# klkuhlm/unconfined

Hardware: AMD Instinct MI355X
Metric: (t,r) drawdown points/sec, Neuman-1974 1024x256 sweep; max |rel err| vs CPU ref (higher is better)
Workload: dtype f64

## Files before the change

unconfined_amd/csrc/ucf_device.h:

```cpp

#include "ucf_math.h"
#include "ucf_plan.h"
#include <type_traits>

namespace UCF_NS {

using namespace ucfm;

#define UCF_STR_(x) #x
#define UCF_STR(x) UCF_STR_(x)
#define UCF_PI 3.14159265358979323846
#define UCF_EPS 2.220446049250313e-16

UCF_DEV double shfl_down1(double v) { return __shfl_down(v, 1, 64); }
UCF_DEV double shift_down1(double x)
{
    const int lo = __double2loint(x), hi = __double2hiint(x);
    const int l2 = __builtin_amdgcn_update_dpp(lo, lo, 0x130, 0xf, 0xf, false);
    const int h2 = __builtin_amdgcn_update_dpp(hi, hi, 0x130, 0xf, 0xf, false);
    return __hiloint2double(h2, l2);
}
UCF_DEV cplx shfl_down1(cplx v) { return cmake(shift_down1(v.re), shift_down1(v.im)); }
UCF_DEV cplx bcast0(cplx v) { return cmake(__shfl(v.re, 0, 64), __shfl(v.im, 0, 64)); }
UCF_DEV double wave_max(double v)
// ... 608 lines not shown
#if UCF_FAST && UCF_DH_PACK
UCF_DEV cplx lane_gather(cplx v, int src) { return cmake(__shfl(v.re, src, 64), __shfl(v.im, src, 64)); }
template <int W>
UCF_DEV cplx qd_quotient_groups(cplx qn, cplx enn, cplx enew, bool valid, int lane)
{
    const double m = fmax(fabs(enew.re), fabs(enew.im));
    const unsigned long long bal = __builtin_amdgcn_ballot_w64(valid && !(m < 1.0e150 && m > 1.0e-150));
    const double r = fast_rcp(__builtin_fma(enew.re, enew.re, enew.im * enew.im));
    const cplx num = cmul(qn, enn);
    cplx res = cmake((num.re * enew.re + num.im * enew.im) * r, (num.im * enew.re - num.re * enew.im) * r);
    if (__builtin_expect(bal != 0, 0)) {
        const bool mine = ((bal >> (lane & ~(W - 1))) & ((1ull << W) - 1)) != 0;
        const cplx scaled = cdiv(cmul(qn, enn), enew);
        if (mine) res = scaled;
    }
    return res;
}
template <int W>
UCF_DEV void qd_step(cplx& q, cplx& en, int r, int M, int lane, bool occ, lds_c* dcol, int pitch)
{
    const int l = lane & (W - 1);
    const cplx qn = shfl_down1(q);
    const cplx enew = cadd(csub(qn, q), en);
    if (l == 0 && occ) {
        dcol[(size_t)(2 * r - 1) * pitch] = make_double2(-q.re, -q.im);
        dcol[(size_t)(2 * r) * pitch] = make_double2(-enew.re, -enew.im);
    }
    if (r < M) {
        const cplx enn = shfl_down1(enew);
        const bool valid = occ && l <= 2 * (M - r - 1) + 1;
        if constexpr (W == UCF_WAVE) q = qd_quotient(qn, enn, enew, valid);
        else q = qd_quotient_groups<W>(qn, enn, enew, valid, lane);
        en = enn;
    }
}
UCF_DEV void dehoog_qd_tile(const ucf_dev_params& P, int lane, int ncur, const double* __restrict__ tD4, lds_c* lds, lds_c* tileB,
                            int pitch, int* zflag, ucf_stats* st)
{
    const int M = P.M, np = P.np;
    const int r32 = (M - 15 > 1) ? M - 15 : 1, r16 = (M - 7 > 1) ? M - 7 : 1;
    const cplx c0 = cmake(0.0, 0.0);
    for (int tq = 0; tq < ncur; tq += 2) {
        cplx Qq = c0, Qe = c0;
        int present = 0;
        for (int hf = 0; hf < 2 && tq + hf < ncur; hf++) {
            const int tt = tq + hf;
            const double tee = 2.0 * tD4[tt];
            const double sigma = P.alpha - P.logtol / (2.0 * tee);
            cplx tl = c0;
            if (lane < np) { const lds_c v = lds[lane * pitch + tt]; tl = cmake(v.x, v.y); }
            const cplx p = cmake(sigma, UCF_PI * lane / tee);
            cplx Pq = c0, Pe = c0;
            for (int which = 0; which < 2; which++) {
                lds_c* col = (which ? tileB : lds) + tt;
                cplx q;
                const bool some = qd_start(which ? cmul(tl, p) : tl, M, lane, st, col, &q);
                const bool live = __builtin_amdgcn_ballot_w64(some) != 0;
                if (lane == 0) zflag[2 * tt + which] = !live;
                if (!live) continue;
                cplx en = c0;
                for (int r = 1; r < r32; r++) qd_step<UCF_WAVE>(q, en, r, M, lane, true, col, pitch);
                present |= 1 << (2 * hf + which);
                const cplx gq = lane_gather(q, lane & 31), ge = lane_gather(en, lane & 31);
                if ((lane >> 5) == which) { Pq = gq; Pe = ge; }
            }
            if (((present >> (2 * hf)) & 3) == 0) continue;
            {
                const int g = lane >> 5;
                const bool occ = (present >> (2 * hf + g)) & 1;
                lds_c* col = (g ? tileB : lds) + tt;
                for (int r = r32; r < r16; r++) qd_step<32>(Pq, Pe, r, M, lane, occ, col, pitch);
                const int src = ((lane >> 4) & 1) * 32 + (lane & 15);
                const cplx gq = lane_gather(Pq, src), ge = lane_gather(Pe, src);
                if ((lane >> 5) == hf) { Qq = gq; Qe = ge; }
            }
        }
        if (present == 0) continue;
        const int g = lane >> 4;
        const bool occ = (present >> g) & 1;
        lds_c* col = ((g & 1) ? tileB : lds) + tq + (g >> 1);
        for (int r = r16; r <= M; r++) qd_step<16>(Qq, Qe, r, M, lane, occ, col, pitch);
    }
}
#endif

UCF_DEV double dehoog_cf_lane(const lds_c* dcol, int pitch, int M, double alpha, double logtol, double t, double tee)
{
    const double gamma = alpha - logtol / (2.0 * tee);
    const lds_c v0 = dcol[0];
    const cplx d0 = cmake(v0.x, v0.y);
    cplx Am2 = cmake(0.0, 0.0), Am1 = d0, Bm2 = cmake(1.0, 0.0), Bm1 = cmake(1.0, 0.0);
    const cplx z = cexp_(cdivr(cscale(cscale(cmake(0.0, 1.0), UCF_PI), t), tee));
    for (int n = 1; n <= 2 * M - 1; n++) {
        const lds_c v = dcol[(size_t)n * pitch];
        const cplx d = cmake(v.x, v.y);
        const cplx An = cadd(Am1, cmul(cmul(d, Am2), z));
        const cplx Bn = cadd(Bm1, cmul(cmul(d, Bm2), z));
        Am2 = Am1; Am1 = An; Bm2 = Bm1; Bm1 = Bn;
    }
    const lds_c vq = dcol[(size_t)(2 * M - 1) * pitch], ve = dcol[(size_t)(2 * M) * pitch];
    const cplx dlast_q = cmake(vq.x, vq.y), dlast_e = cmake(ve.x, ve.y);
    const cplx brem = cdivr(radd(1.0, cmul(csub(dlast_q, dlast_e), z)), 2.0);
    const cplx inner = csqrt_(radd(1.0, cdiv(cmul(dlast_e, z), cmul(brem, brem))));
    const cplx rem = cneg(cmul(brem, rsub(1.0, inner)));
    const cplx A2M = cadd(Am1, cmul(rem, Am2));
    const cplx B2M = cadd(Bm1, cmul(rem, Bm2));
    return exp(gamma * t) / tee * cdiv(A2M, B2M).re;
}

template <int G>
UCF_DEV void shift_down_sets(const cplx (&in)[G], cplx (&out)[G], int lane)
{
#pragma unroll
    for (int g = 0; g < G; g++) {
        const cplx a = shfl_down1(in[g]);
        const cplx nx = (g + 1 < G) ? bcast0(in[g + 1 < G ? g + 1 : g]) : a;
        out[g] = (lane == 63 && g + 1 < G) ? nx : a;
    }
}

template <int G>
UCF_DEV double dehoog_sets(const cplx (&f)[G], int M, double alpha, double logtol, double t, double tee, int lane,
                           ucf_stats* st)
{
    const int n2 = 2 * M;
    double mag = 0.0;
    cplx ff[G], q[G], e[G];
    bool nans[G];
#pragma unroll
    for (int g = 0; g < G; g++) {
        const int i = lane + 64 * g;
        const bool act = i <= n2;
        double m1 = act ? cabs_(f[g]) : 0.0;
        if (d_isnan(m1)) m1 = 0.0;
        mag = fmax(mag, m1);
        const bool nanp = act && (d_isnan(f[g].re) || d_isnan(f[g].im));
        nans[g] = nanp;
        ff[g] = (nanp || !act) ? cmake(act ? 0.0 : 1.0, 0.0) : f[g];
    }
    const double mx = wave_max(mag);
    if (!(mx > UCF_DBL_MIN)) {
        if (st) stat_add(&st->zero_vectors, lane == 0);
        return 0.0;
    }
    if (st) {
#pragma unroll
        for (int g = 0; g < G; g++) stat_add(&st->nan_scrubbed, nans[g]);
    }
    const double gamma = alpha - logtol / (2.0 * tee);
    const cplx ff0 = bcast0(ff[0]);
    const cplx d0 = cdivr(ff0, 2.0);
    cplx fn[G];
    shift_down_sets<G>(ff, fn, lane);
#pragma unroll
    for (int g = 0; g < G; g++) {
        const int i = lane + 64 * g;
        q[g] = (i == 0) ? cdiv(fn[g], d0) : cdiv(fn[g], ff[g]);
        if (i > n2 - 1) q[g] = cmake(1.0, 0.0);
        e[g] = cmake(0.0, 0.0);
    }
    cplx Am2 = cmake(0.0, 0.0), Am1 = d0, Bm2 = cmake(1.0, 0.0), Bm1 = cmake(1.0, 0.0);
    const cplx z = cexp_(cdivr(cscale(cscale(cmake(0.0, 1.0), UCF_PI), t), tee));
    cplx dlast_q = cmake(0.0, 0.0), dlast_e = cmake(0.0, 0.0);
    for (int r = 1; r <= M; r++) {
        cplx qn[G], en[G], enew[G];
        shift_down_sets<G>(q, qn, lane);
        shift_down_sets<G>(e, en, lane);
#pragma unroll
        for (int g = 0; g < G; g++) {
            const int i = lane + 64 * g;
            enew[g] = cadd(csub(qn[g], q[g]), en[g]);
            if (i > 2 * (M - r)) enew[g] = cmake(1.0, 0.0);
        }
        const cplx dq = cneg(bcast0(q[0]));
        const cplx de = cneg(bcast0(enew[0]));
        {
            cplx An = cadd(Am1, cmul(cmul(dq, Am2), z));
            cplx Bn = cadd(Bm1, cmul(cmul(dq, Bm2), z));
            Am2 = Am1; Am1 = An; Bm2 = Bm1; Bm1 = Bn;
        }
        if (r < M) {
            cplx An = cadd(Am1, cmul(cmul(de, Am2), z));
            cplx Bn = cadd(Bm1, cmul(cmul(de, Bm2), z));
            Am2 = Am1; Am1 = An; Bm2 = Bm1; Bm1 = Bn;
            cplx enn[G];
            shift_down_sets<G>(enew, enn, lane);
#pragma unroll
            for (int g = 0; g < G; g++) {
                const int i = lane + 64 * g;
                q[g] = cdiv(cmul(qn[g], enn[g]), enew[g]);
                if (i > 2 * (M - r - 1) + 1) q[g] = cmake(1.0, 0.0);
// ... 824 lines not shown
                } else {
                    cplx acc = cadd(lds_ld(accCur, z, lane), cscale(val, P.tab_premul ? 1.0 : P.gl_w[m]));
                    if (m == ngl - 1) {
                        const double lob = P.j0z[sv + jj - 1] / rD;
                        const double hib = P.j0z[sv + jj] / rD;
                        acc = rscale((hib - lob) / 2.0, acc);
                        areas[(size_t)(jj * nz + z) * UCF_WAVE + lane] = make_double2(acc.re, acc.im);
                        acc = cmake(0.0, 0.0);
                    }
                    lds_st(accCur, z, lane, acc);
                }
            }
            if (!ts && ++m == ngl) { m = 0; jj++; }
        }
        for (int s = 0; s < (R + 1) * nz; s++) sti[(size_t)s * UCF_WAVE + lane] = lds[s * UCF_WAVE + lane];
        if (lane == 0) ndone[pt] = nabs;
    }
}

template <int LAYOUT, int PART, bool WREG, int MODE = 0>
__global__ void __launch_bounds__(UCF_WAVE, (LAYOUT == 0 || (WREG && MODE != 1)) ? 3 : 4)
finish_kernel(const ucf_dev_params P, int npts, int per_point, int nr, int nsv, int svmin,
              const double* __restrict__ tDv, const double* __restrict__ rDv, const int* __restrict__ svv,
              double* __restrict__ hout, double* __restrict__ dhout, ucf_stats* st, int nt, int ir0,
              double2* __restrict__ totlap, const double2* __restrict__ state, const int* __restrict__ ndone, int* __restrict__ defer)
{
    extern __shared__ lds_c lds[];
    const int lane = threadIdx.x;
    const int nz = P.nz, R = P.R, nacc = P.nacc;
    const int nabs = P.N + nacc * P.ngl;
    lds_c* accTS = lds;
    lds_c* scr = lds + (size_t)R * nz * UCF_WAVE;
    const int nloop = (MODE == 2) ? defer[0] : npts;
    for (int wi = blockIdx.x; wi < nloop; wi += gridDim.x) {
        const int pt = (MODE == 2) ? defer[1 + wi] / nz : wi;
        const int zsel = (MODE == 2) ? defer[1 + wi] % nz : 0;
        if (MODE != 2 && ndone[pt] < nabs) continue;
        const work_item W = decode_item<LAYOUT>(P, pt, lane, per_point, nr, nt, ir0, npts);
        const double tD = tDv[W.it], rD = rDv[W.ir];
        const int sv = (LAYOUT == 1) ? svmin : svv[W.it];
        const double tee = 2.0 * tD;
        const double sigma = P.alpha - P.logtol / (2.0 * tee);
        const cplx p = cmake(sigma, UCF_PI * W.mlap / tee);
        const double arg = P.j0z[sv - 1] / rD;
        const double2* __restrict__ sti = state + (size_t)pt * state_slots(P) * UCF_WAVE;
        for (int s = 0; s < R * nz; s++) lds[s * UCF_WAVE + lane] = sti[(size_t)s * UCF_WAVE + lane];
        finish_item<LAYOUT, PART, WREG, MODE>(P, accTS, scr, nullptr, sti + (size_t)(R + 1) * nz * UCF_WAVE, arg, W, pt, tD, tee, p, st, nt, ir0,
                                              totlap, hout, dhout, zsel, (MODE == 2) ? zsel + 1 : nz, (MODE == 1) ? defer : nullptr);
    }
}

#ifndef UCF_DH_TILE
#define UCF_DH_TILE 4
#endif
#if UCF_TU_HAS(1) || UCF_TU_HAS(3)
#ifndef UCF_DH_WAVES
#define UCF_DH_WAVES 4
#endif
template <int TU, bool BIG>
__global__ void __launch_bounds__(UCF_WAVE, BIG ? 4 : UCF_DH_WAVES)
dehoog_tiles_kernel(const ucf_dev_params P, int nt, int nr, int ir0, int nrc, const double* __restrict__ tDv,
                    const double2* __restrict__ totlap, double* __restrict__ hout, double* __restrict__ dhout,
                    ucf_stats* st)
{
    extern __shared__ lds_c lds[];
    const int lane = threadIdx.x;
    const int nz = P.nz, np = P.np;
    const int ntile = (nt + UCF_DH_TILE - 1) / UCF_DH_TILE;
    const long long nwork = (long long)nrc * ntile;
    const int pitch = UCF_DH_TILE + 1;
    lds_c* tileB = lds + (size_t)np * pitch;
    int* zflag = (int*)(tileB + (size_t)np * pitch);
    for (long long w = blockIdx.x; w < nwork; w += gridDim.x) {
        const int irl = (int)(w / ntile), it0 = (int)(w % ntile) * UCF_DH_TILE;
        const int ncur = (nt - it0 < UCF_DH_TILE) ? nt - it0 : UCF_DH_TILE;
        for (int z = 0; z < nz; z++) {
            const double2* src = totlap + ((size_t)irl * nz + z) * np * nt;
            for (int e = lane; e < np * UCF_DH_TILE; e += UCF_WAVE) {
                const int m = e / UCF_DH_TILE, tt = e % UCF_DH_TILE;
                if (tt < ncur) lds[m * pitch + tt] = src[(size_t)m * nt + it0 + tt];
            }
            __syncthreads();
            if constexpr (!BIG) {
#if UCF_FAST && UCF_DH_PACK
                dehoog_qd_tile(P, lane, ncur, tDv + it0, lds, tileB, pitch, zflag, st);
#else
                for (int tt = 0; tt < ncur; tt++) {
                    const double tD = tDv[it0 + tt];
                    const double tee = 2.0 * tD;
                    const double sigma = P.alpha - P.logtol / (2.0 * tee);
                    cplx tl = cmake(0.0, 0.0);
                    if (lane < np) { const lds_c v = lds[lane * pitch + tt]; tl = cmake(v.x, v.y); }
                    const cplx p = cmake(sigma, UCF_PI * lane / tee);
                    bool z0, z1;
                    dehoog_qd_wave(tl, P.M, lane, st, &z0, lds + tt, pitch);
                    dehoog_qd_wave(cmul(tl, p), P.M, lane, st, &z1, tileB + tt, pitch);
                    if (lane == 0) { zflag[2 * tt] = z0; zflag[2 * tt + 1] = z1; }
                }
#endif
                __syncthreads();
                if (lane < 2 * ncur) {
                    const int tt = lane >> 1, which = lane & 1;
                    const int it = it0 + tt;
                    const double tD = tDv[it];
                    double val = 0.0;
                    if (!zflag[lane]) val = dehoog_cf_lane((which ? tileB : lds) + tt, pitch, P.M, P.alpha, P.logtol, tD, 2.0 * tD);
                    const size_t o = ((size_t)it * nr + ir0 + irl) * P.nz_out + P.z_off + z;
                    if (which) dhout[o] = val * tD;
                    else hout[o] = val;
                }
            } else {
                for (int tt = 0; tt < ncur; tt++) {
                    const int it = it0 + tt;
                    const double tD = tDv[it];
                    const double tee = 2.0 * tD;
                    const double sigma = P.alpha - P.logtol / (2.0 * tee);
                    double hval, dval;
                    auto ld = [&](int i) { const lds_c v = lds[i * pitch + tt]; return cmake(v.x, v.y); };
                    if (np <= 2 * UCF_WAVE) dehoog_big<2>(ld, np, P.M, P.alpha, P.logtol, sigma, tD, tee, lane, st, &hval, &dval);
                    else dehoog_big<4>(ld, np, P.M, P.alpha, P.logtol, sigma, tD, tee, lane, st, &hval, &dval);
                    if (lane == 0) {
                        const size_t o = ((size_t)it * nr + ir0 + irl) * P.nz_out + P.z_off + z;
                        hout[o] = hval;
                        dhout[o] = dval;
                    }
                }
            }
            __syncthreads();
        }
    }
}

#endif

#if UCF_TU_HAS(2)
__global__ void __launch_bounds__(UCF_WAVE)
dehoog_points_kernel(const ucf_dev_params P, long long npc, int flat, int per_point, int nr, int ir0, int nrc,
                     const double* __restrict__ tDv, const double2* __restrict__ totlap, double* __restrict__ hout,
                     double* __restrict__ dhout, ucf_stats* st)
{
    const int lane = threadIdx.x;
    const int nz = P.nz;
    for (long long lp = blockIdx.x; lp < npc; lp += gridDim.x) {
        int it;
        size_t obase;
        if (flat) {
            it = per_point ? (int)lp : (int)(lp / nr);
            obase = (size_t)lp;
        } else {
            it = (int)(lp / nrc);
            obase = (size_t)it * nr + ir0 + (int)(lp % nrc);
        }
        const double tD = tDv[it];
        const double tee = 2.0 * tD;
        const double sigma = P.alpha - P.logtol / (2.0 * tee);
        for (int z = 0; z < nz; z++) {
            const double2* src = totlap + ((size_t)lp * nz + z) * P.np;
            double hval, dval;
            if (P.np <= UCF_WAVE) {
                const cplx p = cmake(sigma, UCF_PI * lane / tee);
                cplx tl = cmake(0.0, 0.0);
                if (lane < P.np) { const double2 v = src[lane]; tl = cmake(v.x, v.y); }
                hval = dehoog_wave(tl, P.M, P.alpha, P.logtol, tD, tee, lane, st);
                dval = dehoog_wave(cmul(tl, p), P.M, P.alpha, P.logtol, tD, tee, lane, st) * tD;
            } else {
                auto ld = [&](int i) { const double2 v = src[i]; return cmake(v.x, v.y); };
                if (P.np <= 2 * UCF_WAVE) dehoog_big<2>(ld, P.np, P.M, P.alpha, P.logtol, sigma, tD, tee, lane, st, &hval, &dval);
                else dehoog_big<4>(ld, P.np, P.M, P.alpha, P.logtol, sigma, tD, tee, lane, st, &hval, &dval);
            }
            if (lane == 0) {
                hout[obase * P.nz_out + P.z_off + z] = hval;
                dhout[obase * P.nz_out + P.z_off + z] = dval;
            }
        }
    }
}

#endif

template <int FAMILY>
__global__ void __launch_bounds__(UCF_WAVE)
samples_kernel(const ucf_dev_params P, int n_a, const double* __restrict__ av, double rD,
               const double* __restrict__ pv, double* __restrict__ fp)
{
    extern __shared__ lds_c lds[];
    const int lane = threadIdx.x;
    const int ia = blockIdx.x;
    if (ia >= n_a) return;
    const bool live = lane < P.np;
    const cplx p = live ? cmake(pv[2 * lane], pv[2 * lane + 1]) : cmake(1.0, 0.0);
    const double a = av[ia];
    bool need_lay1 = false;
    for (int z = 0; z < P.nz; z++) need_lay1 |= (P.zLay[z] == 1);
// ... 195 lines not shown
```

unconfined_amd/csrc/ucf_fastpath.h:

```cpp
#pragma once

namespace UCF_NS {

#define UCF_UNIFORM_BLOCK() asm volatile("" ::: "memory")
#define UCF_UNIFORM_BLOCK_F(FAMILY) do { if constexpr ((FAMILY) != 4) UCF_UNIFORM_BLOCK(); } while (0)

struct fprim {
    double ch, sh, ei, sn, cs;
};

template <bool POS, bool SMALLY = false>
UCF_DEV fprim prim_from_e(double x, double ax, double e, double ei, double y, const sc_ctx& sc)
{
    const int salt = sc.salt;
    fprim f;
    f.ei = ei;
    const double he = 0.5 * e;
    f.ch = __builtin_fma(0.5, ei, he);
    double s;
    if (ax < 0.35) {
        const double x2 = ax * ax;
        double pl = addk(mulk(x2, UCF_KHERE(1.0 / 6227020800.0, salt)), UCF_KHERE(1.0 / 39916800.0, salt));
        pl = fmak(pl, x2, UCF_KHERE(1.0 / 362880.0, salt));
        pl = fmak(pl, x2, UCF_KHERE(1.0 / 5040.0, salt));
// ... 74 lines not shown
    const double xz = xc * zD;
    const double e = exp_tab_(xc, sc), ez = exp_tab_(xz, sc);
    const double r = fast_rcp(e * ez);
    *f = prim_from_e<true, true>(xc, xc, e, r * ez, y, sc);
    *fz = prim_from_e<true, true>(xz, xz, ez, r * e, y * zD, sc);
}

UCF_DEV cplx cfma(cplx a, cplx b, cplx c)
{
    return cmake(__builtin_fma(a.re, b.re, __builtin_fma(-a.im, b.im, c.re)), __builtin_fma(a.re, b.im, __builtin_fma(a.im, b.re, c.im)));
}
UCF_DEV cplx cfnma(cplx a, cplx b, cplx c)
{
    return cmake(__builtin_fma(-a.re, b.re, __builtin_fma(a.im, b.im, c.re)), __builtin_fma(-a.re, b.im, __builtin_fma(-a.im, b.re, c.im)));
}
UCF_DEV cplx cinv_plain(cplx z)
{
    const double r = fast_rcp(z.re * z.re + z.im * z.im);
    return cmake(z.re * r, -(z.im * r));
}
UCF_DEV cplx cinv_scaled(cplx z)
{
    const double m = fmax(fabs(z.re), fabs(z.im));
    const int il = __builtin_amdgcn_frexp_exp(m) - 1;
    const double c = ldexp(z.re, -il), d = ldexp(z.im, -il);
    const double r = fast_rcp(c * c + d * d);
    return cmake(ldexp(c * r, -il), ldexp(-(d * r), -il));
}

UCF_DEV cplx cinv_auto(cplx z)
{
    const double m = fmax(fabs(z.re), fabs(z.im));
    if (__builtin_amdgcn_ballot_w64(!(m < 1.0e150 && m > 1.0e-150)) == 0) return cinv_plain(z);
    return cinv_scaled(z);
}

struct lane_consts {
    cplx p, lt, xifac;
    cplx fdB1;
    cplx mnpv;
};

UCF_DEV lane_consts make_lane_consts(const ucf_dev_params& P, cplx p, cplx lt)
{
    lane_consts L;
    L.p = p;
    L.lt = lt;
    cplx xf = rscale(P.alphaD, cinv_plain(p));
    if (P.model == 3) {
        cplx sum = cmake(0.0, 0.0);
        for (int j = 0; j < P.MoenchM; j++) sum = cadd(sum, cinv_plain(radd(1.0, cscale(p, P.MoenchInvGamma[j]))));
        xf = cmul(cscale(xf, (double)P.MoenchM), cinv_plain(sum));
    }
    L.xifac = xf;
    L.fdB1 = cscale(cscale(cscale(p, P.fd_beta0), P.fd_expmb2), P.inv_kappa);
    L.mnpv = radd(1.0, cscale(p, P.mn_vartheta * P.mn_c3));
    return L;
}

struct fast_common {
    sc_ctx sc;
    cplx th, eta, ff1, ff2, inv_she, she, che, top, g3, inv_den, ex1;
    cplx chz0;
    fprim p1;
    int have_p1;
    cplx mn_uod;
#ifdef UCF_SINGLE_RCP
    cplx q, den;
#endif
    cplx fd_s1;
    cplx top3, fd_s13;
    bool small_eta, fd_use, fd_use3;
    int any_small, any_large;
};

template <int FAMILY>
UCF_DEV double fast_scale(const ucf_dev_params& P)
{
    if (FAMILY == 0 || FAMILY == 3) return 2.0;
    if (FAMILY == 5) return P.inv_bD;
    return (FAMILY == 2 && P.model == 4) ? 2.0 : 2.0 * P.inv_bD;
}

template <int FAMILY, bool PAIR = false>
UCF_DEV bool fast_eta(const ucf_dev_params& P, const lane_consts& L, double a, fast_common& S)
{
    const double a2 = a * a;
    const cplx q = caddr(L.p, a2);
#ifdef UCF_SINGLE_RCP
    S.q = q;
#endif
    double mq = 0.0;
    if (PAIR && FAMILY != 0) {
        double r;
        rsq_pair(q.re * q.re + q.im * q.im, &mq, &r);
        S.th = cmake(q.re * r, -(q.im * r));
    } else {
        const double r = fast_rcp(q.re * q.re + q.im * q.im);
        S.th = cmake(q.re * r, -(q.im * r));
    }
    if (FAMILY == 0) return q.re > 0.0;
    {
        const double qr = q.re * P.inv_kappa, qi = q.im * P.inv_kappa;
        double r, hr;
        const double d = PAIR ? mq * P.inv_kappa : sqrt_only(__builtin_fma(qr, qr, qi * qi));
        sqrt_hrsqrt(0.5 * (d + qr), &r, &hr);
        S.eta = cmake(r, qi * hr);
    }
    return (S.eta.re <= P.fast_eta_max) & (q.re > 0.0) & (fabs(S.eta.im) < P.fast_im_max);
}
template <int FAMILY, bool PAIR = false>
UCF_DEV bool fast_eta_wave(const ucf_dev_params& P, const lane_consts& L, double a, fast_common& S)
{
    (void)fast_eta<FAMILY, PAIR>(P, L, a, S);
    const cplx q = caddr(L.p, a * a);
    unsigned long long bad = __builtin_amdgcn_ballot_w64(!(q.re > 0.0));
    if (FAMILY != 0) {
        bad |= __builtin_amdgcn_ballot_w64(!(S.eta.re <= P.fast_eta_max));
        bad |= __builtin_amdgcn_ballot_w64(!(fabs(S.eta.im) < P.fast_im_max));
    }
    return bad == 0;
}

#ifndef UCF_ZPAIR_PHASES
#define UCF_ZPAIR_PHASES 3
#endif
#ifndef UCF_ZPAIR_INTERVALS
#define UCF_ZPAIR_INTERVALS 1
#endif
enum {
    UCF_PH_RANGE = 1,
    UCF_PH_IM = 2,
    UCF_PH_LARGE = 4,
    UCF_PH_YS = 8,
    UCF_PH_YL = 16
};
UCF_DEV int zpair_part_phase(const ucf_dev_params& P, const lane_consts& L, double a_max)
{
    if (!(UCF_ZPAIR_PHASES & 2)) return 0;
    const double lim = 0.99 * P.fast_eta_max;
    const bool ok = (L.p.re > 0.0) & (lim > 0.0) & ((__builtin_fma(a_max, a_max, fabs(L.p.re) + fabs(L.p.im)) * P.inv_kappa) < lim * lim);
    return __builtin_amdgcn_ballot_w64(!ok) == 0 ? UCF_PH_RANGE : 0;
}
template <bool UNI>
UCF_DEV bool fast_eta_wave_zpair(const ucf_dev_params& P, const lane_consts& L, double a, fast_common& S, int& ph, int may_set)
{
    if constexpr (!UNI) return fast_eta_wave<2, true>(P, L, a, S);
    (void)fast_eta<2, true>(P, L, a, S);
    unsigned long long bad = 0;
    if (!(ph & UCF_PH_RANGE)) {
        const cplx q = caddr(L.p, a * a);
        bad |= __builtin_amdgcn_ballot_w64(!(q.re > 0.0));
        bad |= __builtin_amdgcn_ballot_w64(!(S.eta.re <= P.fast_eta_max));
        UCF_UNIFORM_BLOCK();
    }
    if (!(ph & UCF_PH_IM)) {
        const double ai = fabs(S.eta.im);
        bad |= __builtin_amdgcn_ballot_w64(!(ai < P.fast_im_max));
        if ((UCF_ZPAIR_PHASES & 2) && may_set && __builtin_amdgcn_ballot_w64(!(ai < 0.5 * P.fast_im_max)) == 0) ph |= UCF_PH_IM;
        UCF_UNIFORM_BLOCK();
    }
    return bad == 0;
}

template <int FAMILY, bool FOLD = false, bool LAY3 = true, bool LAY1 = true, bool NOFOLD = false, bool ZPAIR = false>
UCF_DEV void fast_common_terms(const ucf_dev_params& P, const lane_consts& L, double a, bool need_lay1_in, fast_common& S,
                               bool need_lay3_in = false, bool need_lay12 = true)
{
    static_assert(!ZPAIR || (FOLD && FAMILY == 2), "ZPAIR: folded water-table kernels only");
    const double a2 = a * a;
    if (FAMILY == 0) return;
    if (FAMILY == 3) {
        const fprim p1 = prim<true>(S.eta.re, S.eta.im, S.sc);
        S.che = pcosh(p1);
        S.she = psinh(p1);
        const double wr = __builtin_fma(a2, P.mn_c3, L.mnpv.re), wi = L.mnpv.im;
        double vr, hr;
        sqrt_hrsqrt(0.5 * (sqrt_only(__builtin_fma(wr, wr, wi * wi)) + wr), &vr, &hr);
        const cplx u = cmake(P.mn_u0 * (1.0 - vr), -(P.mn_u0 * (wi * hr)));
        const cplx Delta0 = cfnma(u, S.che, cmul(S.eta, S.she));
        S.mn_uod = cmul(u, cinv_auto(Delta0));
        return;
    }
    const bool hantush = NOFOLD || !(FAMILY == 2 && P.model == 4);
// ... 350 lines not shown
```

unconfined_amd/csrc/ucf_launch_plan.h:

```cpp
#pragma once
#include "../../include/ucf.h"
#include "ucf_env.h"

#define UCF_WAVE 64
#define UCF_MAX_R 16
#define UCF_LDS_C 16

struct ucf_dev_params {
    int model, MNtype, order, timeType, MoenchM;
    int M, np, k, N, R, nacc, ngl, nz;
    int tab_premul;
    int nj0z, any_lay3;
    int any_lay1;
    int any_fold;
    int nz_out, z_off;
    double timePar[2];
    double kappa, alphaD, beta;
    double lD, dD, bD, dD1, lD1;
    double MoenchInvGamma[UCF_MAX_MOENCH];
    double alpha, logtol, maxexp;
    double inv_kappa, inv_bD, fast_eta_max, fast_im_max;
    int fold_dD, fold_lD1, share_g1top, _pad2;
    double g1_delta;
    double hs_rDw, hs_CDw, hs_tDb;
    double mn_vartheta, mn_u0, mn_c3;
    double fd_h, fd_invhsq, fd_beta0, fd_beta3, fd_expmb2;
    double fd_isk, fd_gmax;
    double hv[UCF_MAX_R];
    double zD[UCF_MAX_NZ];
    int zLay[UCF_MAX_NZ];
    const double* ts_x;
    const double* ts_w;
    const double* gl_x;
    const double* gl_w;
    const double* j0z;
    const double* fd_e;
    const double* sched;
    const double* sc_tab;
};
#define UCF_SC_ENTRIES (256 + 128)
#define UCF_IWPB 4

#define UCF_PART 16
#define UCF_WYNN_REGS 12

#ifndef UCF_FOLD_WAVES
#define UCF_FOLD_WAVES 5
#endif
#ifndef UCF_UNFOLD_WAVES
#define UCF_UNFOLD_WAVES 4
#endif
#ifndef UCF_TAIL_LSPLIT_DEFAULT
#define UCF_TAIL_LSPLIT_DEFAULT 3
#endif
#ifndef UCF_NZC
#define UCF_NZC(F, FO) (LAYOUT == 1 && (F) == 2 && (FO) ? 1 : 0)
#endif
#ifndef UCF_NZC2
#define UCF_NZC2(F, FO) ((LAYOUT == 1 || LAYOUT == 3) ? 2 : 0)
#endif

static inline int family_of(const ucf_dev_params& dp)
{
    switch (dp.model) {
    case 0: return 0;
    case 1: return 1;
    case 2: return 5;
    case 3: case 4: case 5: return 2;
    case 6: return dp.MNtype == 1 ? 3 : (dp.MNtype == 2 ? 4 : -1);
    default: return -1;
    }
}

static inline bool areas_in_lds(const ucf_dev_params& dp)
{
    const size_t with_areas = ((size_t)(dp.R + 1 + dp.nacc) * dp.nz * UCF_WAVE + (size_t)(2 * dp.nacc > dp.R ? 2 * dp.nacc : dp.R) * UCF_PART) * UCF_LDS_C;
    return with_areas <= 20 * 1024;
}

static inline size_t point_lds_bytes(const ucf_dev_params& dp, bool fast, bool resume = false)
{
    size_t bytes = ((size_t)(dp.R + 1 + ((areas_in_lds(dp) && !resume) ? dp.nacc : 0)) * dp.nz * UCF_WAVE + (size_t)(2 * dp.nacc > dp.R ? 2 * dp.nacc : dp.R) * UCF_PART) * UCF_LDS_C;
    if (!fast && family_of(dp) == 4) bytes += 2 * (size_t)dp.order * UCF_WAVE * UCF_LDS_C;
    return bytes;
}

static inline size_t samples_lds_bytes(const ucf_dev_params& dp, bool fast)
{
    if (fast) return UCF_SC_ENTRIES * UCF_LDS_C;
    return family_of(dp) == 4 ? 2 * (size_t)dp.order * UCF_WAVE * UCF_LDS_C : 16;
}

static inline int split_kind(const ucf_dev_params& dp, bool fast)
{
    const int fam = family_of(dp);
    if (fast) {
        if (fam >= 0 && fam <= 5) return 1;
    } else if (fam == 4 && 2 * (size_t)dp.order * UCF_WAVE * UCF_LDS_C > 16 * 1024) return 0;
    return 2;
}

struct ucf_transform_buffers {
    size_t ndone, todo, defer, wcount;
    size_t ints;
    size_t state_item_bytes;
    size_t ltab;
    size_t state_bytes;
};
static inline ucf_transform_buffers transform_buffers(const ucf_dev_params& dp, bool fast, size_t nwork, size_t lt_rows)
{
    const int kind = split_kind(dp, fast);
    ucf_transform_buffers b;
    b.ndone = 0;
    b.todo = b.ndone + nwork;
    b.defer = b.todo + 1 + nwork;
    b.wcount = b.defer + 1 + nwork * (size_t)dp.nz;
    b.ints = b.wcount + 2;
    b.state_item_bytes = kind ? (size_t)(dp.R + 1 + dp.nacc) * dp.nz * UCF_WAVE * UCF_LDS_C : 0;
    b.ltab = nwork * b.state_item_bytes;
    b.state_bytes = b.ltab + (kind == 1 ? lt_rows * dp.np * UCF_LDS_C : 0);
    return b;
// ... 123 lines not shown
```

unconfined_amd/csrc/ucf_plan.cpp:

```cpp
#include <cfloat>
#include <cmath>
#include <cstdlib>
#include <cstring>
#include <new>
#include <vector>

#include "ucf_host.h"

using namespace ucf_host;

namespace {

void j0_zeros(int n, double* z)
{
    const double PI = 4.0 * std::atan(1.0);
    for (int i = 0; i < n; i++) {
        double x = (i + 0.75) * PI;
        for (int it = 0; it < 100; it++) {
            const double dx = j0(x) / j1(x);
            x = x + dx;
            if (std::fabs(dx) < std::nextafter(std::fabs(x), INFINITY) - std::fabs(x)) break;
        }
        z[i] = x;
    }
// ... 121 lines not shown
        {
            const double K = (dp.fd_invhsq - dp.fd_beta3 / h) * dp.fd_invhsq;
            dp.fd_isk = (K > 0.0 && std::isfinite(K)) ? 1.0 / std::sqrt(K) : 0.0;
            dp.fd_gmax = std::exp2(500.0 / (double)P.order) - 1.0;
        }
    }
    if (P.model == 2) {
        const double PI = 4.0 * std::atan(1.0);
        dp.hs_rDw = D.rDw;
        dp.hs_CDw = D.rDw * D.rDw / (2.0 * (D.l_eff - D.d_eff) * P.Ss);
        dp.hs_tDb = PI * (D.rDwobs * D.rDwobs) / (P.sF * P.Ss);
    }
    if (P.model == 6 && P.MNtype == 1) {
        const double beta0 = P.ak * P.b;
        const double phiDa = P.psia / P.b, phiDk = P.psik / P.b;
        dp.mn_vartheta = beta0 * P.Sy / (P.Ss * P.b) * std::exp(-(beta0 * (phiDa - phiDk)));
        dp.mn_u0 = beta0 / 2.0;
        dp.mn_c3 = 1.0 / (P.kappa * dp.mn_u0 * dp.mn_u0);
    }

    std::vector<double> sched;
    if (P.timeType < 0) {
        const bool linear = P.timeType <= -101;
        const int n = linear ? -P.timeType - 100 : -P.timeType;
        sched.resize(2 * n + 2);
        double prev = 0.0, sum = 0.0, yprev = 0.0;
        for (int k = 0; k < n; k++) {
            double cur = P.timeParExt[n + 1 + k];
            if (linear) {
                const double denom = P.timeParExt[k + 1] - P.timeParExt[k];
                const double w = (cur - yprev) / denom;
                yprev = cur;
                cur = w;
            }
            const double dq = cur - prev;
            prev = cur;
            sched[k] = P.timeParExt[k];
            sched[n + k] = dq;
            sum = (k == 0) ? dq : sum + dq;
        }
        sched[2 * n] = P.timeParExt[n];
        sched[2 * n + 1] = sum;
    }
    if (create) {
        const size_t n_tab = (size_t)N + (size_t)R * N + 2 * (size_t)ngl + D.nj0z + fd_e.size() + sched.size() + 1 + 2 * UCF_SC_ENTRIES;
        std::vector<double> host(n_tab);
        size_t o = 0;
        pl->o_tsx = o; std::memcpy(&host[o], pl->h_ts_x, sizeof(double) * N); o += N;
        pl->o_tsw = o; std::memcpy(&host[o], pl->h_ts_w, sizeof(double) * (size_t)R * N); o += (size_t)R * N;
        pl->o_glx = o; std::memcpy(&host[o], pl->h_gl_x, sizeof(double) * ngl); o += ngl;
        pl->o_glw = o; std::memcpy(&host[o], pl->h_gl_w, sizeof(double) * ngl); o += ngl;
        pl->o_j0z = o; std::memcpy(&host[o], pl->h_j0z, sizeof(double) * D.nj0z); o += D.nj0z;
        pl->o_fde = o; if (!fd_e.empty()) std::memcpy(&host[o], fd_e.data(), sizeof(double) * fd_e.size());
        o += fd_e.size();
        pl->o_sched = o; if (!sched.empty()) std::memcpy(&host[o], sched.data(), sizeof(double) * sched.size());
        o += sched.size();
        o += (o & 1);
        pl->o_sct = o; sincos_table(&host[o]); exp2_table(&host[o + 512]);
        pl->tables_bytes = n_tab * sizeof(double);
        if (hipMalloc((void**)&pl->d_tables, pl->tables_bytes) != hipSuccess)
            return fail(UCF_ERR_NOMEM, "hipMalloc of %zu table bytes failed", pl->tables_bytes);
        if (hipMemcpy(pl->d_tables, host.data(), pl->tables_bytes, hipMemcpyHostToDevice) != hipSuccess)
            return fail(UCF_ERR_HIP, "table upload failed");
    } else if (!fd_e.empty() || !sched.empty()) {
        {
            std::lock_guard<std::mutex> g(pl->mu);
            for (ucf_workspace* w : pl->ws) (void)hipStreamSynchronize((hipStream_t)w->stream);
        }
        if (!fd_e.empty() && hipMemcpy(pl->d_tables + pl->o_fde, fd_e.data(), sizeof(double) * fd_e.size(), hipMemcpyHostToDevice) != hipSuccess)
            return fail(UCF_ERR_HIP, "table upload failed");
        if (!sched.empty() && hipMemcpy(pl->d_tables + pl->o_sched, sched.data(), sizeof(double) * sched.size(), hipMemcpyHostToDevice) != hipSuccess)
            return fail(UCF_ERR_HIP, "table upload failed");
    }

    dp.model = P.model; dp.MNtype = P.MNtype; dp.order = P.order; dp.timeType = P.timeType; dp.MoenchM = P.MoenchM;
    dp.M = P.M; dp.np = D.np; dp.k = P.k; dp.N = N; dp.R = R; dp.nacc = P.nacc; dp.ngl = ngl; dp.nz = 0;
    dp.nj0z = D.nj0z;
    dp.timePar[0] = P.timePar[0]; dp.timePar[1] = P.timePar[1];
    dp.kappa = P.kappa; dp.alphaD = D.alphaD; dp.beta = P.beta;
    dp.lD = D.lD; dp.dD = D.dD; dp.bD = D.bD; dp.dD1 = 1.0 - D.dD; dp.lD1 = 1.0 - D.lD;
    for (int m = 0; m < P.MoenchM; m++) dp.MoenchInvGamma[m] = 1.0 / D.MoenchGamma[m];
    dp.alpha = P.alpha; dp.logtol = std::log(P.tol); dp.maxexp = -std::log(DBL_EPSILON) / 3.0;
    dp.inv_kappa = 1.0 / P.kappa;
    dp.inv_bD = 1.0 / D.bD;
    dp.fold_dD = (D.dD == 0.0);
    dp.fold_lD1 = (dp.lD1 == 0.0);
    dp.g1_delta = (dp.dD1 - 1.0) + D.dD;
    dp.share_g1top = (dp.g1_delta == 0.0) ? 1 : (std::fabs(dp.g1_delta) < 1.0e-15 ? 2 : 0);
    dp.fast_eta_max = (dp.fold_dD && dp.fold_lD1) ? 700.0 : 350.0;
    dp.ts_x = pl->d_tables + pl->o_tsx;
    dp.ts_w = pl->d_tables + pl->o_tsw;
    dp.gl_x = pl->d_tables + pl->o_glx;
    dp.gl_w = pl->d_tables + pl->o_glw;
    dp.j0z = pl->d_tables + pl->o_j0z;
    dp.fd_e = pl->d_tables + pl->o_fde;
    dp.sched = pl->d_tables + pl->o_sched;
    dp.sc_tab = pl->d_tables + pl->o_sct;
    return UCF_OK;
}

const char** names_scratch(ucf_workspace* ws) { return ws->tm_names; }
}

namespace ucf_host {

int validate(const ucf_params& P)
{
    if (P.model < 0 || P.model > 6) return fail(UCF_ERR_INVALID_MODEL, "invalid model choice %d (valid: 0..6)", P.model);
    if (P.model == 3 && P.MoenchM < 1) return fail(UCF_ERR_MOENCH, "number of Moench alphas must be >= 1 for model 3");
    if (P.MoenchM > UCF_MAX_MOENCH) return fail(UCF_ERR_MOENCH, "more than %d Moench alphas", UCF_MAX_MOENCH);
    if (P.model > 0 && (P.gammaSkin < 0.0 || P.d < 0.0 || P.l < 0.0))
        return fail(UCF_ERR_GEOMETRY, "negative geometry parameters (gamma, d, l)");
    if (P.b <= 0.0 || P.Kr <= 0.0 || P.Ss <= 0.0) return fail(UCF_ERR_AQUIFER, "zero or negative aquifer parameters (b, Kr, Ss)");
    if (P.model > 2 && (P.kappa <= 0.0 || P.Sy <= 0.0))
        return fail(UCF_ERR_AQUIFER, "zero or negative unconfined aquifer parameters (kappa, Sy)");
    double l = P.l, d = P.d;
    if (P.MNtype == 1) {
        if (std::fabs(l - P.b) > FLT_EPSILON) l = P.b;
        if (d > FLT_EPSILON) d = 0.0;
    }
    if (P.model > 0 && d >= l) return fail(UCF_ERR_GEOMETRY, "screen top/bottom: l must be > d (l=%g d=%g)", l, d);
    if (P.model == 6) {
        if (P.ac < 0.0 || P.ak < 0.0 || P.usL < 0.0 || P.psia < 0.0 || P.psik < 0.0)
            return fail(UCF_ERR_MISHRA_NEUMAN, "invalid Mishra/Neuman parameters (a_c, a_k, L, psi_a, psi_k)");
        if (P.MNtype == 2 && P.order < 3) return fail(UCF_ERR_MISHRA_NEUMAN, "Mishra/Neuman finite difference order must be >= 3");
        if (P.MNtype == 0)
            return fail(UCF_ERR_UNSUPPORTED, "Mishra/Neuman type 0 is the quad-precision ARB path, excluded from this build");
        if (P.MNtype < 0 || P.MNtype > 2) return fail(UCF_ERR_MISHRA_NEUMAN, "invalid Mishra/Neuman solution type %d", P.MNtype);
    }
    if ((P.model == 4 || P.model == 5) && P.beta < 0.0) return fail(UCF_ERR_MALAMA_BETA, "Malama beta cannot be negative");
    if (P.model == 3)
        for (int i = 0; i < P.MoenchM; i++)
            if (P.MoenchAlpha[i] < 0.0) return fail(UCF_ERR_MOENCH, "Moench alphas cannot be negative");
    if (P.M < 2) return fail(UCF_ERR_DEHOOG, "de Hoog M must be >= 2 (M=%d)", P.M);
    if (P.M > UCF_MAX_LAP_M) return fail(UCF_ERR_UNSUPPORTED, "de Hoog M=%d: the wave-cooperative inversion holds at most four Laplace samples per lane (M <= %d)", P.M, UCF_MAX_LAP_M);
    if (P.k - P.R < 2) return fail(UCF_ERR_TANH_SINH, "tanh-sinh k (%d) too low for %d Richardson levels", P.k, P.R);
    if (P.R < 1) return fail(UCF_ERR_TANH_SINH, "Richardson extrapolation level must be >= 1");
    if (P.R > UCF_MAX_R || P.k > 20) return fail(UCF_ERR_UNSUPPORTED, "tanh-sinh k=%d R=%d beyond build limits", P.k, P.R);
    if (P.j0s[0] < 1 || P.j0s[1] < 1 || P.nacc < 1 || P.k < 1)
        return fail(UCF_ERR_GAUSS_LOBATTO, "min/max split, # accelerated terms and k must be >= 1");
    if (P.ord < 3) return fail(UCF_ERR_GAUSS_LOBATTO, "Gauss-Lobatto order must be >= 3");
    if (P.model == 2 && (P.rwobs <= 0.0 || P.sF <= 0.0))
        return fail(UCF_ERR_OBSERVATION, "model 2 needs a positive observation-well radius and shape factor");
    if (P.timeType == 0 || P.timeType > 8 || P.timeType < -(100 + UCF_MAX_SCHEDULE))
        return fail(UCF_ERR_UNSUPPORTED, "time behaviour %d does not exist (1..8, -1..-100 piecewise constant, -101..-%d piecewise linear)", P.timeType, 100 + UCF_MAX_SCHEDULE);
    if (P.timeType <= -101) {
        const int n = -P.timeType - 100;
        for (int k = 0; k < n; k++) {
            const double denom = P.timeParExt[k + 1] - P.timeParExt[k];
            if (std::fabs(denom) < (double)FLT_EPSILON)
                return fail(UCF_ERR_BAD_ARGUMENT, "no vertical sloped lines in piecewise linear pumping rate (knots %d and %d coincide)", k + 1, k + 2);
        }
    }
    return UCF_OK;
}

void nondimensionalise(const ucf_params& P, ucf_derived& D)
{
    const double PI = 4.0 * std::atan(1.0);
    std::memset(&D, 0, sizeof(D));
    double l = P.l, d = P.d, ac = P.ac;
    if (P.MNtype == 1) {
        if (std::fabs(P.ac - P.ak) > FLT_EPSILON) ac = P.ak;
        if (std::fabs(l - P.b) > FLT_EPSILON) l = P.b;
        if (d > FLT_EPSILON) d = 0.0;
    }
// ... 324 lines not shown
```

Before: 9.217 million.

## Add slot-based qd tile with ballot-guarded fast division and split CF lanes

Adds a new de Hoog qd-table builder that replaces the per-step scaled complex division with a fast reciprocal. It uses a wave ballot to fall back to the safe division only when magnitudes leave a safe range, and DPP shifts with bound_ctrl zero fill. The continued-fraction evaluation now uses four lanes per time point, with separate lanes computing the A and B recurrences that are exchanged by a shuffle, doubling lane parallelism. It also adds a precomputed half_inv_kappa to fold a scale in the paired eta sqrt. The risks are accuracy loss from the fast reciprocal, and extra shuffles and divergence.

Measured after the change: 9.389 million, median of 6. 1.9% higher.

```diff
diff --git a/unconfined_amd/csrc/ucf_device.h b/unconfined_amd/csrc/ucf_device.h
--- a/unconfined_amd/csrc/ucf_device.h
+++ b/unconfined_amd/csrc/ucf_device.h
@@ -714,6 +714,156 @@
         for (int r = r16; r <= M; r++) qd_step<16>(Qq, Qe, r, M, lane, occ, col, pitch);
     }
 }
+
+#ifndef UCF_DH_SLOTS
+#define UCF_DH_SLOTS 1
+#endif
+#if UCF_DH_SLOTS
+UCF_DEV double shift_down1_new(double x)
+{
+    const int lo = __double2loint(x), hi = __double2hiint(x);
+    const int l2 = __builtin_amdgcn_update_dpp(0, lo, 0x130, 0xf, 0xf, true);
+    const int h2 = __builtin_amdgcn_update_dpp(0, hi, 0x130, 0xf, 0xf, true);
+    return __hiloint2double(h2, l2);
+}
+UCF_DEV cplx shift_down1_new(cplx v) { return cmake(shift_down1_new(v.re), shift_down1_new(v.im)); }
+template <int W>
+UCF_DEV unsigned long long qd_valid_lanes(int r, int M)
+{
+    const unsigned long long b = (1ull << (2 * (M - r))) - 1ull;
+    if constexpr (W == 32) return b | (b << 32);
+    if constexpr (W == 16) return b * 0x0001000100010001ull;
+    return b;
+}
+template <int W>
+UCF_DEV void qd_slot_step(cplx q, cplx en, cplx& q2, cplx& en2, unsigned long long vmask, bool st0, lds_c* drow, int pitch, int lane)
+{
+    const cplx qn = shift_down1_new(q);
+    const cplx enew = cadd(csub(qn, q), en);
+    if (st0) {
+        drow[0] = make_double2(q.re, q.im);
+        drow[pitch] = make_double2(enew.re, enew.im);
+    }
+    const cplx enn = shift_down1_new(enew);
+    double m;
+    asm("v_max_f64 %0, |%1|, |%2|" : "=v"(m) : "v"(enew.re), "v"(enew.im));
+    const unsigned long long bal = (__builtin_amdgcn_ballot_w64(!(m < 1.0e150)) | __builtin_amdgcn_ballot_w64(!(m > 1.0e-150))) & vmask;
+    en2 = enn;
+    if (W == UCF_WAVE && bal != 0) {
+        q2 = cdiv(cmul(qn, enn), enew);
+        return;
+    }
+    const double rc = fast_rcp(__builtin_fma(enew.re, enew.re, enew.im * enew.im));
+    const cplx num = cmul(qn, enn);
+    q2 = cmake((num.re * enew.re + num.im * enew.im) * rc, (num.im * enew.re - num.re * enew.im) * rc);
+    if (W != UCF_WAVE && __builtin_expect(bal != 0, 0)) {
+        const bool mine = ((bal >> (lane & ~(W - 1) & 63)) & ((1ull << (W & 63)) - 1)) != 0;
+        const cplx scaled = cdiv(cmul(qn, enn), enew);
+        if (mine) q2 = scaled;
+    }
+}
+template <int W>
+UCF_DEV void qd_slot_steps(cplx& q, cplx& en, int r0, int r1, int M, unsigned long long occ_lanes, bool st0, lds_c* col, int pitch, int lane)
+{
+    lds_c* drow = col + (size_t)(2 * r0 - 1) * pitch;
+    int r = r0;
+    for (; r + 1 < r1; r += 2) {
+        cplx qb, eb;
+        qd_slot_step<W>(q, en, qb, eb, qd_valid_lanes<W>(r, M) & occ_lanes, st0, drow, pitch, lane);
+        qd_slot_step<W>(qb, eb, q, en, qd_valid_lanes<W>(r + 1, M) & occ_lanes, st0, drow + 2 * pitch, pitch, lane);
+        drow += 4 * pitch;
+    }
+    if (r < r1) {
+        cplx qb, eb;
+        qd_slot_step<W>(q, en, qb, eb, qd_valid_lanes<W>(r, M) & occ_lanes, st0, drow, pitch, lane);
+        q = qb; en = eb;
+    }
+}
+UCF_DEV bool qd_start_slots(cplx f, int M, int lane, ucf_stats* st, lds_c* dcol, cplx* q1)
+{
+    const int n2 = 2 * M;
+    const bool act = lane <= n2;
+    double mag = act ? fmax(fabs(f.re), fabs(f.im)) : 0.0;
+    if (d_isnan(mag)) mag = 0.0;
+    double mx = wave_max(mag);
+    if (__builtin_expect(!(mx > UCF_DBL_MIN) && mx > 0.7 * UCF_DBL_MIN, 0)) {
+        mag = act ? cabs_(f) : 0.0;
+        if (d_isnan(mag)) mag = 0.0;
+        mx = wave_max(mag);
+    }
+    if (!(mx > UCF_DBL_MIN)) {
+        if (st) stat_add(&st->zero_vectors, lane == 0);
+        return false;
+    }
+    const bool nanp = act && (d_isnan(f.re) || d_isnan(f.im));
+    if (st) stat_add(&st->nan_scrubbed, nanp);
+    cplx ff = (nanp || !act) ? cmake(act ? 0.0 : 1.0, 0.0) : f;
+    const cplx ff0 = bcast0(ff);
+    const cplx d0 = cdivr(ff0, 2.0);
+    if (lane == 0) dcol[0] = make_double2(d0.re, d0.im);
+    const cplx fnext = shift_down1_new(ff);
+    *q1 = cdiv(fnext, (lane == 0) ? d0 : ff);
+    return true;
+}
+UCF_DEV void dehoog_qd_tile_slots(const ucf_dev_params& P, int lane, int ncur, const double* __restrict__ tD4, lds_c* lds, lds_c* tileB,
+                                  int pitch, int* zflag, ucf_stats* st)
+{
+    const int M = P.M, np = P.np;
+    const int r32 = (M - 15 > 1) ? M - 15 : 1, r16 = (M - 7 > 1) ? M - 7 : 1;
+    const cplx c0 = cmake(0.0, 0.0);
+    for (int tq = 0; tq < ncur; tq += 2) {
+        cplx Qq = c0, Qe = c0;
+        int present = 0;
+        for (int hf = 0; hf < 2 && tq + hf < ncur; hf++) {
+            const int tt = tq + hf;
+            const double tee = 2.0 * tD4[tt];
+            const double sigma = P.alpha - P.logtol / (2.0 * tee);
+            cplx tl = c0;
+            if (lane < np) { const lds_c v = lds[lane * pitch + tt]; tl = cmake(v.x, v.y); }
+            const cplx p = cmake(sigma, UCF_PI * lane / tee);
+            cplx Pq = c0, Pe = c0;
+            for (int which = 0; which < 2; which++) {
+                lds_c* col = (which ? tileB : lds) + tt;
+                cplx q;
+                const bool some = qd_start_slots(which ? cmul(tl, p) : tl, M, lane, st, col, &q);
+                const bool live = __builtin_amdgcn_ballot_w64(some) != 0;
+                if (lane == 0) zflag[2 * tt + which] = !live;
+                if (!live) continue;
+                cplx en = c0;
+                qd_slot_steps<UCF_WAVE>(q, en, 1, r32, M, ~0ull, lane == 0, col, pitch, lane);
+                present |= 1 << (2 * hf + which);
+                const cplx gq = lane_gather(q, lane & 31), ge = lane_gather(en, lane & 31);
+                if ((lane >> 5) == which) { Pq = gq; Pe = ge; }
+            }
+            const int pr = (present >> (2 * hf)) & 3;
+            if (pr == 0) continue;
+            {
+                const int g = lane >> 5;
+                const unsigned long long occ_lanes = ((pr & 1) ? 0xffffffffull : 0ull) | ((pr & 2) ? 0xffffffff00000000ull : 0ull);
+                lds_c* col = (g ? tileB : lds) + tt;
+                qd_slot_steps<32>(Pq, Pe, r32, r16, M, occ_lanes, (lane & 31) == 0 && ((pr >> g) & 1), col, pitch, lane);
+                const int src = ((lane >> 4) & 1) * 32 + (lane & 15);
+                const cplx gq = lane_gather(Pq, src), ge = lane_gather(Pe, src);
+                if ((lane >> 5) == hf) { Qq = gq; Qe = ge; }
+            }
+        }
+        if (present == 0) continue;
+        const int g = lane >> 4;
+        unsigned long long occ_lanes = 0ull;
+#pragma unroll
+        for (int k = 0; k < 4; k++) occ_lanes |= ((present >> k) & 1) ? (0xffffull << (16 * k)) : 0ull;
+        const bool st0 = (lane & 15) == 0 && ((present >> g) & 1);
+        lds_c* col = ((g & 1) ? tileB : lds) + tq + (g >> 1);
+        qd_slot_steps<16>(Qq, Qe, r16, M, M, occ_lanes, st0, col, pitch, lane);
+        const cplx qn = shift_down1_new(Qq);
+        const cplx enew = cadd(csub(qn, Qq), Qe);
+        if (st0) {
+            col[(size_t)(2 * M - 1) * pitch] = make_double2(Qq.re, Qq.im);
+            col[(size_t)(2 * M) * pitch] = make_double2(enew.re, enew.im);
+        }
+    }
+}
+#endif
 #endif
 
 UCF_DEV double dehoog_cf_lane(const lds_c* dcol, int pitch, int M, double alpha, double logtol, double t, double tee)
@@ -739,6 +889,36 @@
     const cplx B2M = cadd(Bm1, cmul(rem, Bm2));
     return exp(gamma * t) / tee * cdiv(A2M, B2M).re;
 }
+
+#if UCF_FAST && UCF_DH_PACK && UCF_DH_SLOTS
+UCF_DEV double dehoog_cf_slot(const lds_c* dcol, int pitch, int M, double alpha, double logtol, double t, double tee, int ab)
+{
+    const double gamma = alpha - logtol / (2.0 * tee);
+    const lds_c v0 = dcol[0];
+    const cplx d0 = cmake(v0.x, v0.y);
+    cplx Xm2 = cmake(ab ? 1.0 : 0.0, 0.0), Xm1 = ab ? cmake(1.0, 0.0) : d0;
+    const cplx z = cexp_(cdivr(cscale(cscale(cmake(0.0, 1.0), UCF_PI), t), tee));
+    auto next = [&](int n, cplx xm1, cplx xm2) {
+        const lds_c v = dcol[(size_t)n * pitch];
+        return cadd(xm1, cmul(cmul(cmake(-v.x, -v.y), xm2), z));
+    };
+    int n = 1;
+    for (; n + 1 <= 2 * M - 1; n += 2) {
+        Xm2 = next(n, Xm1, Xm2);
+        Xm1 = next(n + 1, Xm2, Xm1);
+    }
+    if (n <= 2 * M - 1) { const cplx Xn = next(n, Xm1, Xm2); Xm2 = Xm1; Xm1 = Xn; }
+    const lds_c vq = dcol[(size_t)(2 * M - 1) * pitch], ve = dcol[(size_t)(2 * M) * pitch];
+    const cplx dlast_q = cmake(-vq.x, -vq.y), dlast_e = cmake(-ve.x, -ve.y);
+    const cplx brem = cdivr(radd(1.0, cmul(csub(dlast_q, dlast_e), z)), 2.0);
+    const cplx inner = csqrt_(radd(1.0, cdiv(cmul(dlast_e, z), cmul(brem, brem))));
+    const cplx rem = cneg(cmul(brem, rsub(1.0, inner)));
+    const cplx X2M = cadd(Xm1, cmul(rem, Xm2));
+    const cplx other = cmake(__shfl_xor(X2M.re, 1, 64), __shfl_xor(X2M.im, 1, 64));
+    const cplx A2M = ab ? other : X2M, B2M = ab ? X2M : other;
+    return exp(gamma * t) / tee * cdiv(A2M, B2M).re;
+}
+#endif
 
 template <int G>
 UCF_DEV void shift_down_sets(const cplx (&in)[G], cplx (&out)[G], int lane)
@@ -1729,7 +1909,9 @@
             }
             __syncthreads();
             if constexpr (!BIG) {
-#if UCF_FAST && UCF_DH_PACK
+#if UCF_FAST && UCF_DH_PACK && UCF_DH_SLOTS
+                dehoog_qd_tile_slots(P, lane, ncur, tDv + it0, lds, tileB, pitch, zflag, st);
+#elif UCF_FAST && UCF_DH_PACK
                 dehoog_qd_tile(P, lane, ncur, tDv + it0, lds, tileB, pitch, zflag, st);
 #else
                 for (int tt = 0; tt < ncur; tt++) {
@@ -1746,6 +1928,20 @@
                 }
 #endif
                 __syncthreads();
+#if UCF_FAST && UCF_DH_PACK && UCF_DH_SLOTS
+                if (lane < 4 * ncur) {
+                    const int tt = lane >> 2, which = (lane >> 1) & 1;
+                    const int it = it0 + tt;
+                    const double tD = tDv[it];
+                    double val = 0.0;
+                    if (!zflag[lane >> 1]) val = dehoog_cf_slot((which ? tileB : lds) + tt, pitch, P.M, P.alpha, P.logtol, tD, 2.0 * tD, lane & 1);
+                    const size_t o = ((size_t)it * nr + ir0 + irl) * P.nz_out + P.z_off + z;
+                    if ((lane & 1) == 0) {
+                        if (which) dhout[o] = val * tD;
+                        else hout[o] = val;
+                    }
+                }
+#else
                 if (lane < 2 * ncur) {
                     const int tt = lane >> 1, which = lane & 1;
                     const int it = it0 + tt;
@@ -1756,6 +1952,7 @@
                     if (which) dhout[o] = val * tD;
                     else hout[o] = val;
                 }
+#endif
             } else {
                 for (int tt = 0; tt < ncur; tt++) {
                     const int it = it0 + tt;
diff --git a/unconfined_amd/csrc/ucf_fastpath.h b/unconfined_amd/csrc/ucf_fastpath.h
--- a/unconfined_amd/csrc/ucf_fastpath.h
+++ b/unconfined_amd/csrc/ucf_fastpath.h
@@ -180,6 +180,9 @@
     return (FAMILY == 2 && P.model == 4) ? 2.0 : 2.0 * P.inv_bD;
 }
 
+#ifndef UCF_ZPAIR_HALFK
+#define UCF_ZPAIR_HALFK 1
+#endif
 template <int FAMILY, bool PAIR = false>
 UCF_DEV bool fast_eta(const ucf_dev_params& P, const lane_consts& L, double a, fast_common& S)
 {
@@ -198,6 +201,14 @@
         S.th = cmake(q.re * r, -(q.im * r));
     }
     if (FAMILY == 0) return q.re > 0.0;
+#if UCF_ZPAIR_HALFK
+    if (PAIR) {
+        const double qi = q.im * P.inv_kappa;
+        double r, hr;
+        sqrt_hrsqrt(__builtin_fma(q.re, P.half_inv_kappa, mq * P.half_inv_kappa), &r, &hr);
+        S.eta = cmake(r, qi * hr);
+    } else
+#endif
     {
         const double qr = q.re * P.inv_kappa, qi = q.im * P.inv_kappa;
         double r, hr;
diff --git a/unconfined_amd/csrc/ucf_launch_plan.h b/unconfined_amd/csrc/ucf_launch_plan.h
--- a/unconfined_amd/csrc/ucf_launch_plan.h
+++ b/unconfined_amd/csrc/ucf_launch_plan.h
@@ -37,6 +37,7 @@
     const double* fd_e;
     const double* sched;
     const double* sc_tab;
+    double half_inv_kappa;
 };
 #define UCF_SC_ENTRIES (256 + 128)
 #define UCF_IWPB 4
diff --git a/unconfined_amd/csrc/ucf_plan.cpp b/unconfined_amd/csrc/ucf_plan.cpp
--- a/unconfined_amd/csrc/ucf_plan.cpp
+++ b/unconfined_amd/csrc/ucf_plan.cpp
@@ -227,6 +227,7 @@
     for (int m = 0; m < P.MoenchM; m++) dp.MoenchInvGamma[m] = 1.0 / D.MoenchGamma[m];
     dp.alpha = P.alpha; dp.logtol = std::log(P.tol); dp.maxexp = -std::log(DBL_EPSILON) / 3.0;
     dp.inv_kappa = 1.0 / P.kappa;
+    dp.half_inv_kappa = 0.5 * dp.inv_kappa;
     dp.inv_bD = 1.0 / D.bD;
     dp.fold_dD = (D.dD == 0.0);
     dp.fold_lD1 = (dp.lD1 == 0.0);
```
